# Arthur151/ROMP

Measured on NVIDIA H100. Metric: frames/sec 512x512 ROMP-HRNet32 (whole hot path), higher is better.
Workload: dtype bf16

## Files before the change

romp_b200/csrc/conv_tc.cu:

```cuda
#include <mutex>

#include "conv_tc.cuh"
#include "tc_device.cuh"

namespace b200romp {

thread_local int g_tc_pdl_override = -1;

constexpr int kTcThreads = 384;
constexpr int kMaxRings = 2;

__host__ __device__ constexpr int s2_row_bytes(int cin, int eb) { return cin * eb >= 512 ? 64 : (cin * eb < 128 ? cin * eb : 128); }

__host__ __device__ constexpr int tc_num_rings(int stages) { return stages >= 4 ? kMaxRings : 1; }
__host__ __device__ constexpr int tc_ring_size(int stages, int ring) { return tc_num_rings(stages) == 1 ? stages : (stages + 1 - ring) / 2; }
__host__ __device__ constexpr int tc_ring_base(int stages, int ring) { return ring ? (stages + 1) / 2 : 0; }

template <int MODE, int CIN, int NT, int EB>
struct TcCfg {
  static constexpr bool S2 = MODE == 2;
  static constexpr int KS = MODE == 1 ? 1 : 3;
  static constexpr int TAPS = KS * KS;
  static constexpr int PAD = KS / 2;
  static constexpr int ROWB = S2 ? s2_row_bytes(CIN, EB) : tc_row_bytes(KS, CIN, EB);
  static constexpr int CW = ROWB / EB;
  static constexpr int KCH = CIN / CW;
  static constexpr int KSTEPS = ROWB / 32;
  static constexpr uint32_t LAYOUT = tc_layout(ROWB);
  static constexpr int HW_ = 8 + 2 * PAD;
  static constexpr int HH = 16 + 2 * PAD;
  __host__ __device__ static constexpr int BH(int i) { return i < 2 ? 17 : 16; }
  __host__ __device__ static constexpr int BW(int i) { return (i & 1) ? 8 : 9; }
  __host__ __device__ static constexpr int SUB_BYTES(int i) { return (BH(i) * BW(i) * ROWB + 1023) / 1024 * 1024; }
  __host__ __device__ static constexpr int SUB_OFF(int i) { return i == 0 ? 0 : SUB_OFF(i - 1) + SUB_BYTES(i - 1); }
  static constexpr int STAGE_PAYLOAD = S2 ? (17 * 9 + 17 * 8 + 16 * 9 + 16 * 8) * ROWB : HH * HW_ * ROWB;
  static constexpr int STAGE_BYTES = S2 ? SUB_OFF(3) + SUB_BYTES(3) : (STAGE_PAYLOAD + 1023) / 1024 * 1024;
  static constexpr int BTILE = NT * ROWB;
  static constexpr int B_BYTES = TAPS * KCH * BTILE;
  static constexpr bool FOLDABLE = MODE == 3 && CIN == 64 && NT == 64 && EB == 2;
};

template <int MODE, int CIN, int NT, int EB, bool GENERIC>
__global__ void __launch_bounds__(kTcThreads, 1)
conv_tc_kernel(const __grid_constant__ CUtensorMap tmap, const __grid_constant__ S2Maps s2maps, const ConvParams p,
               const uint8_t* __restrict__ wpack, int tiles_x, int tiles_y, int num_tiles, int stages, unsigned kmask) {
  using Cfg = TcCfg<MODE, CIN, NT, EB>;
  extern __shared__ uint8_t smem_raw[];
  uint8_t* smem = reinterpret_cast<uint8_t*>((reinterpret_cast<uintptr_t>(smem_raw) + 1023) & ~(uintptr_t)1023);
  uint8_t* sB = smem;
  uint8_t* sA = smem + Cfg::B_BYTES;
  uint64_t* full = reinterpret_cast<uint64_t*>(sA + (size_t)stages * Cfg::STAGE_BYTES);
  uint64_t* empty = full + stages;
  uint64_t* b_full = empty + stages;

  const int warp = threadIdx.x >> 5;
  if (threadIdx.x == 0) {
    for (int i = 0; i < stages; ++i) {
      mbar_init(&full[i], 1);
      mbar_init(&empty[i], 4);
    }
    mbar_init(b_full, 1);
    fence_barrier_init();
  }
  __syncthreads();
  pdl_trigger();
  const int per_frame = tiles_x * tiles_y;
  const int nrings = tc_num_rings(stages);

  if (warp == 0) {
    if (elect_one()) {
      mbar_arrive_expect_tx(b_full, Cfg::B_BYTES);
      const uint8_t* wsrc = wpack + (size_t)blockIdx.y * Cfg::B_BYTES;
      for (int i = 0; i < Cfg::TAPS * Cfg::KCH; ++i)
        bulk_copy_g2s(sB + (size_t)i * Cfg::BTILE, wsrc + (size_t)i * Cfg::BTILE, Cfg::BTILE, b_full);
      pdl_wait();
      const uint64_t pol = l2_policy_stream();
      int stage = 0, stage_other = 0;
      uint32_t phase = 0, phase_other = 0;
      int it = 0;
      for (int tile = blockIdx.x; tile < num_tiles; tile += gridDim.x, ++it) {
        const int n = tile / per_frame, rem = tile % per_frame;
        const int y0 = (rem / tiles_x) * 16, x0 = (rem % tiles_x) * 8;
        const int ring = nrings == 2 ? (it & 1) : 0, rbase = tc_ring_base(stages, ring), rsize = tc_ring_size(stages, ring);
        for (int c = 0; c < Cfg::KCH; ++c) {
          const int sidx = rbase + stage;
          mbar_wait(&empty[sidx], phase ^ 1);
          mbar_arrive_expect_tx(&full[sidx], Cfg::STAGE_PAYLOAD);
          uint8_t* dst = sA + (size_t)sidx * Cfg::STAGE_BYTES;
          if constexpr (Cfg::S2) {
#pragma unroll
            for (int i = 0; i < 4; ++i) {
              const int ph = i < 2 ? 1 : 0, pw = (i & 1) ? 0 : 1;
              tma_load_5d(dst + Cfg::SUB_OFF(i), &s2maps.m[i], &full[sidx], pw * p.in_C + p.in_c_off + c * Cfg::CW, x0 - pw, ph,
                          y0 - ph, n, pol);
            }
          } else {
            tma_load_4d(dst, &tmap, &full[sidx], c * Cfg::CW, x0 - Cfg::PAD, y0 - Cfg::PAD, n, pol);
          }
          if (++stage == rsize) { stage = 0; phase ^= 1; }
        }
        if (nrings == 2) { const int ts = stage; stage = stage_other; stage_other = ts; const uint32_t tp = phase; phase = phase_other; phase_other = tp; }
      }
    }
  } else if (warp >= 4 && (warp >> 2) <= nrings) {
    const int g = (warp >> 2) - 1, t = threadIdx.x & 127, wlane = threadIdx.x & 31;
    pdl_wait();
    mbar_wait(b_full, 0);
    const uint32_t b_base = smem_u32(sB);
    const int rbase = tc_ring_base(stages, g), rsize = tc_ring_size(stages, g);
    int stage = 0;
    uint32_t phase = 0;
    for (int tile = blockIdx.x + g * gridDim.x; tile < num_tiles; tile += nrings * gridDim.x) {
      const int n = tile / per_frame, rem = tile % per_frame;
      const int y0 = (rem / tiles_x) * 16, x0 = (rem % tiles_x) * 8;
      float acc[2][NT / 2];
#pragma unroll
      for (int h = 0; h < 2; ++h)
#pragma unroll
        for (int j = 0; j < NT / 2; ++j) acc[h][j] = 0.f;
      uint32_t scale_d = 0;
      int prev = -1;
      for (int c = 0; c < Cfg::KCH; ++c) {
        const int sidx = rbase + stage;
        mbar_wait(&full[sidx], phase);
        uint8_t* a_stage = sA + (size_t)sidx * Cfg::STAGE_BYTES;
        if constexpr (EB == 4) {
          tf32_round_smem(a_stage, Cfg::STAGE_BYTES, t, 128);
          fence_proxy_async();
          wg_bar_sync(1 + g);
        }
        const uint32_t a_base = smem_u32(a_stage);
        wgmma_fence();
#pragma unroll
        for (int tap = 0; tap < Cfg::TAPS; ++tap) {
          const int r = tap / Cfg::KS, s = tap % Cfg::KS;
          uint32_t a_tap, sbo;
          if constexpr (Cfg::S2) {
            const int sub = (r != 1 ? 0 : 2) + (s != 1 ? 0 : 1);
            const int bw = Cfg::BW(sub);
            a_tap = a_base + (uint32_t)(Cfg::SUB_OFF(sub) + ((r == 2 ? bw : 0) + (s == 2 ? 1 : 0)) * Cfg::ROWB);
            sbo = bw * Cfg::ROWB;
          } else {
            a_tap = a_base + (uint32_t)((r * Cfg::HW_ + s) * Cfg::ROWB);
            sbo = Cfg::HW_ * Cfg::ROWB;
          }
          const uint32_t b_tap = b_base + (uint32_t)((tap * Cfg::KCH + c) * Cfg::BTILE);
#pragma unroll
          for (int k = 0; k < Cfg::KSTEPS; ++k) {
            if (Cfg::FOLDABLE && !((kmask >> (tap * 2 + (k * 2) / Cfg::KSTEPS)) & 1u)) continue;
            const uint64_t bdesc = make_smem_desc(b_tap + k * 32, 8 * Cfg::ROWB, Cfg::LAYOUT);
            wgmma_any<NT, EB>(acc[0], make_smem_desc(a_tap + k * 32, sbo, Cfg::LAYOUT), bdesc, scale_d);
            wgmma_any<NT, EB>(acc[1], make_smem_desc(a_tap + 8 * sbo + k * 32, sbo, Cfg::LAYOUT), bdesc, scale_d);
            scale_d = 1;
          }
        }
        wgmma_commit();
        if (prev >= 0) {
          wgmma_wait<1>();
          if (wlane == 0) mbar_arrive(&empty[prev]);
        }
        prev = sidx;
        if (++stage == rsize) { stage = 0; phase ^= 1; }
      }
      wgmma_wait<0>();
      if (wlane == 0) mbar_arrive(&empty[prev]);
      wg_epilogue<NT, GENERIC ? kEpiGeneric : kEpiNhwc>(p, acc, p.bias, n, y0, x0, blockIdx.y * NT, t);
    }
  }
}

PFN_encodeTiled tc_get_encode() {
  static PFN_encodeTiled fn = nullptr;
  static std::once_flag once;
  std::call_once(once, [] {
    void* ptr = nullptr;
    cudaDriverEntryPointQueryResult qres;
    if (cudaGetDriverEntryPoint("cuTensorMapEncodeTiled", &ptr, cudaEnableDefault, &qres) == cudaSuccess &&
        qres == cudaDriverEntryPointSuccess)
      fn = reinterpret_cast<PFN_encodeTiled>(ptr);
  });
  return fn;
}

int tc_encode_tiled(CUtensorMap* map, CUtensorMapDataType dtype, int rank, const void* base, const cuuint64_t* dims,
                    const cuuint64_t* strides, const cuuint32_t* box, CUtensorMapSwizzle swizzle, const char* tag) {
  PFN_encodeTiled encode = tc_get_encode();
  if (!encode) {
    set_error("%s: cuTensorMapEncodeTiled is unavailable", tag);
    return B200ROMP_ECUDA;
  }
  const cuuint32_t estr[5] = {1, 1, 1, 1, 1};
  const CUresult cr = encode(map, dtype, rank, const_cast<void*>(base), dims, strides, box, estr, CU_TENSOR_MAP_INTERLEAVE_NONE,
                             swizzle, CU_TENSOR_MAP_L2_PROMOTION_L2_128B, CU_TENSOR_MAP_FLOAT_OOB_FILL_NONE);
  if (cr != CUDA_SUCCESS) {
    set_error("%s: cuTensorMapEncodeTiled failed with %d", tag, (int)cr);
    return B200ROMP_ECUDA;
  }
  return B200ROMP_OK;
}

int tc_encode_nhwc_input(CUtensorMap* map, const ConvParams& p, int eb, int box_c, int box_w, int box_h, CUtensorMapSwizzle swizzle,
                         const char* tag) {
  const cuuint64_t dims[4] = {(cuuint64_t)p.cin, (cuuint64_t)p.Win, (cuuint64_t)p.Hin, (cuuint64_t)p.B};
  const cuuint64_t strides[3] = {(cuuint64_t)p.in_C * eb, (cuuint64_t)p.Win * p.in_C * eb, (cuuint64_t)p.Hin * p.Win * p.in_C * eb};
  const cuuint32_t box[4] = {(cuuint32_t)box_c, (cuuint32_t)box_w, (cuuint32_t)box_h, 1};
  return tc_encode_tiled(map, eb == 2 ? CU_TENSOR_MAP_DATA_TYPE_BFLOAT16 : CU_TENSOR_MAP_DATA_TYPE_FLOAT32, 4,
                         static_cast<const uint8_t*>(p.in) + (size_t)p.in_c_off * eb, dims, strides, box, swizzle, tag);
}

float tc_round_tf32_host(float w) {
  uint32_t u;
  memcpy(&u, &w, 4);
  if ((u & 0x7F800000u) != 0x7F800000u) u = (u + 0x1000u) & ~0x1FFFu;
  float r;
  memcpy(&r, &u, 4);
  return r;
}

std::vector<uint8_t> tc_pack_image(const float* w_oihw, int cin, int cout, int taps, int nt, int rowb, int eb) {
  const int cw = rowb / eb, kch = cin / cw, ntiles = (cout + nt - 1) / nt, per16 = 16 / eb;
  std::vector<uint8_t> img((size_t)ntiles * taps * kch * nt * rowb, 0);
  for (int j = 0; j < ntiles; ++j)
    for (int t = 0; t < taps; ++t)
      for (int c = 0; c < kch; ++c) {
        uint8_t* tile = img.data() + (((size_t)j * taps + t) * kch + c) * nt * rowb;
        for (int n = 0; n < nt; ++n)
          for (int k = 0; k < cw; ++k) {
            const int co = j * nt + n, ci = c * cw + k;
            if (co >= cout) continue;
            const float w = w_oihw[((size_t)co * cin + ci) * taps + t];
            const int chunk16 = k / per16;
            const int phase = rowb == 128 ? (n & 7) : ((n >> 1) & 3);
            const size_t byte = (size_t)n * rowb + (size_t)((chunk16 ^ phase) * 16) + (k % per16) * eb;
            if (eb == 2) { const __nv_bfloat16 b = __float2bfloat16_rn(w); memcpy(tile + byte, &b, 2); }
            else { const float f = tc_round_tf32_host(w); memcpy(tile + byte, &f, 4); }
          }
      }
  return img;
}

int tc_pack_weights(const float* w_oihw, int cin, int cout, int taps, int nt, void** d_out, std::vector<void*>* allocs, int rowb, int eb) {
  const std::vector<uint8_t> img = tc_pack_image(w_oihw, cin, cout, taps, nt, rowb, eb);
  *d_out = upload(img.data(), img.size(), allocs);
  return *d_out ? B200ROMP_OK : B200ROMP_ECUDA;
}

std::string TcConvPlan::describe() const {
  char buf[128];
  snprintf(buf, sizeof(buf), " [tc%s k%d v%d nt%d grid %dx%d smem %d stages %d%s]", eb == 4 ? "-tf32" : "", kind / 10, kind % 10, nt, grid_x,
           grid_y, smem_bytes, stages, kmask != 0xFFFFFFFFu ? " pixel-pairs" : "");
  return buf;
}

static bool tc_s2_supported(const ConvParams& p) {
  if ((p.in_dtype != B200ROMP_BF16 && p.in_dtype != B200ROMP_F32) || p.input_norm || p.out_nchw || p.pow_channel >= 0) return false;
  const int eb = p.in_dtype == B200ROMP_F32 ? 4 : 2;
  if (eb == 4 && (p.out_dtype != B200ROMP_F32 || (p.res != nullptr && p.res_dtype != B200ROMP_F32))) return false;
  if (p.cin != 32 && p.cin != 64 && p.cin != 128 && p.cin != 256) return false;
  if (eb == 4 && p.cin == 256) return false;
  if (p.in_C % 8 != 0 || p.in_c_off % 8 != 0) return false;
  if (p.cout % 32 != 0 || p.Hin % 2 != 0 || p.Win % 2 != 0) return false;
  if (p.Hout % 16 != 0 || p.Wout % 8 != 0 || p.Hout * 2 != p.Hin || p.Wout * 2 != p.Win) return false;
  if (p.out_C % 8 != 0 || p.out_c_off % 8 != 0) return false;
  if (p.res != nullptr && (p.res_C % 8 != 0 || p.res_c_off % 8 != 0)) return false;
  if ((reinterpret_cast<uintptr_t>(p.in) & 15) != 0) return false;
  return true;
}

static bool tc_shape_supported(const ConvParams& p, int ksize, int stride) {
  if (stride == 2 && ksize == 3) return tc_s2_supported(p);
  if (stride != 1 || (ksize != 1 && ksize != 3)) return false;
  if ((p.in_dtype != B200ROMP_BF16 && p.in_dtype != B200ROMP_F32) || p.input_norm) return false;
  if (p.in_dtype == B200ROMP_F32 && (p.out_dtype != B200ROMP_F32 || (p.res != nullptr && p.res_dtype != B200ROMP_F32))) return false;
  if (p.cin != 32 && p.cin != 64 && p.cin != 128 && p.cin != 256) return false;
  if (p.Hout % 16 != 0 || p.Wout % 8 != 0) return false;
  if (p.in_C % 8 != 0 || p.in_c_off % 8 != 0) return false;
  if (p.out_nchw) {
    if (p.out_dtype != B200ROMP_F32 || p.up != 1 || p.res != nullptr) return false;
    return (reinterpret_cast<uintptr_t>(p.in) & 15) == 0;
  }
  if (p.pow_channel >= 0 || p.cout % 32 != 0) return false;
  if (p.out_C % 8 != 0 || p.out_c_off % 8 != 0) return false;
  if (p.res != nullptr && (p.res_C % 8 != 0 || p.res_c_off % 8 != 0)) return false;
  if ((reinterpret_cast<uintptr_t>(p.in) & 15) != 0) return false;
  return true;
}

static int tc_rowb(int ksize, int stride, int cin, int eb) { return stride == 2 ? s2_row_bytes(cin, eb) : tc_row_bytes(ksize, cin, eb); }

static bool tc_tile(const ConvParams& p, int ksize, int stride, TcConvPlan* plan) {
  const int eb = p.in_dtype == B200ROMP_F32 ? 4 : 2;
  const int rowb = tc_rowb(ksize, stride, p.cin, eb), kch = p.cin / (rowb / eb);
  const int budget = 227 * 1024 - 1024  - 1024 ;
  auto bbytes = [&](int n) { return ksize * ksize * kch * n * rowb; };
  int nt = (p.cout % 64 == 0) ? 64 : 32;
  int stage_bytes, stages;
  if (stride == 2) {
    auto sub_bytes = [&](int i) { return ((i < 2 ? 17 : 16) * ((i & 1) ? 8 : 9) * rowb + 1023) / 1024 * 1024; };
    stage_bytes = sub_bytes(0) + sub_bytes(1) + sub_bytes(2) + sub_bytes(3);
    if (nt == 64 && bbytes(64) + 2 * stage_bytes > budget && bbytes(32) + 2 * stage_bytes <= budget) nt = 32;
    if (nt == 64 && bbytes(64) + stage_bytes > budget) nt = 32;
    if (bbytes(nt) + stage_bytes > budget) return false;
    stages = std::min(4, (budget - bbytes(nt)) / stage_bytes);
  } else {
    const int hh = 16 + 2 * (ksize / 2), hw = 8 + 2 * (ksize / 2);
    stage_bytes = (hh * hw * rowb + 1023) / 1024 * 1024;
    if (bbytes(nt) + 3 * stage_bytes > budget && nt == 64) nt = 32;
    if (bbytes(nt) + 2 * stage_bytes > budget && nt == 32) nt = 16;
    if (bbytes(nt) + 2 * stage_bytes > budget) return false;
    stages = std::min((budget - bbytes(nt)) / stage_bytes, 8);
  }
  plan->kind = stride == 2 ? 32 : ksize * 10;
  plan->eb = eb;
  plan->cin = p.cin; plan->cout = p.cout; plan->nt = nt;
  plan->stages = stages;
  plan->smem_bytes = bbytes(nt) + stages * stage_bytes + 1024 + 1024;
  return true;
}

bool tc_conv_supported(const ConvParams& p, int ksize, int stride) {
  TcConvPlan plan;
  return tc_shape_supported(p, ksize, stride) && tc_tile(p, ksize, stride, &plan);
}

template <int MODE, int CIN, int NT, int EB>
static int launch_inst(const TcConvPlan& plan, const ConvParams& p, cudaStream_t stream, bool set_attr_only) {
  if (set_attr_only) {
    B2R_CUDA_OK(cudaFuncSetAttribute(conv_tc_kernel<MODE, CIN, NT, EB, true>, cudaFuncAttributeMaxDynamicSharedMemorySize, 227 * 1024));
    B2R_CUDA_OK(cudaFuncSetAttribute(conv_tc_kernel<MODE, CIN, NT, EB, false>, cudaFuncAttributeMaxDynamicSharedMemorySize, 227 * 1024));
    return B200ROMP_OK;
  }
  auto kern = p.cout % NT == 0 && tc_nhwc_out(p, p.cout) ? conv_tc_kernel<MODE, CIN, NT, EB, false> : conv_tc_kernel<MODE, CIN, NT, EB, true>;
  const int tiles_x = p.Wout / 8, tiles_y = p.Hout / 16;
  const int num_tiles = tiles_x * tiles_y * p.B;
  dim3 grid(std::min(plan.grid_x, num_tiles), plan.grid_y);
  B2R_CUDA_OK(tc_launch(kern, grid, kTcThreads, plan.smem_bytes, stream, plan.tmap_in, plan.tmap_s2, p,
                        reinterpret_cast<const uint8_t*>(plan.d_wpack), tiles_x, tiles_y, num_tiles, plan.stages, plan.kmask));
  return B200ROMP_OK;
}

static int dispatch(const TcConvPlan& plan, const ConvParams& p, cudaStream_t stream, bool attr) {
  const int mode = plan.kind == 32 ? 2 : plan.kind / 10;
#define B2R_CASE(M, C, N, E) \
  if (mode == M && plan.cin == C && plan.nt == N && plan.eb == E) return launch_inst<M, C, N, E>(plan, p, stream, attr);
  B2R_CASE(3, 32, 32, 2) B2R_CASE(3, 32, 64, 2) B2R_CASE(3, 64, 32, 2) B2R_CASE(3, 64, 64, 2) B2R_CASE(3, 128, 32, 2) B2R_CASE(3, 128, 64, 2)
  B2R_CASE(3, 256, 32, 2) B2R_CASE(3, 256, 64, 2)
  B2R_CASE(1, 32, 32, 2) B2R_CASE(1, 32, 64, 2) B2R_CASE(1, 64, 32, 2) B2R_CASE(1, 64, 64, 2) B2R_CASE(1, 128, 32, 2) B2R_CASE(1, 128, 64, 2)
  B2R_CASE(1, 256, 32, 2) B2R_CASE(1, 256, 64, 2)
  B2R_CASE(2, 32, 32, 2) B2R_CASE(2, 32, 64, 2) B2R_CASE(2, 64, 32, 2) B2R_CASE(2, 64, 64, 2) B2R_CASE(2, 128, 32, 2) B2R_CASE(2, 256, 32, 2)
  B2R_CASE(3, 32, 32, 4) B2R_CASE(3, 32, 64, 4) B2R_CASE(3, 64, 32, 4) B2R_CASE(3, 64, 64, 4) B2R_CASE(3, 128, 32, 4) B2R_CASE(3, 256, 16, 4)
  B2R_CASE(1, 32, 32, 4) B2R_CASE(1, 32, 64, 4) B2R_CASE(1, 64, 32, 4) B2R_CASE(1, 64, 64, 4) B2R_CASE(1, 128, 32, 4) B2R_CASE(1, 128, 64, 4)
  B2R_CASE(1, 256, 32, 4) B2R_CASE(1, 256, 64, 4)
  B2R_CASE(2, 32, 32, 4) B2R_CASE(2, 32, 64, 4) B2R_CASE(2, 64, 32, 4) B2R_CASE(2, 128, 32, 4)
#undef B2R_CASE
  set_error("conv_tc: no instantiation for mode %d cin%d nt%d eb%d", mode, plan.cin, plan.nt, plan.eb);
  return B200ROMP_EINVAL;
}

int tc_conv_prepare(const ConvParams& p, int ksize, int stride, const float* w_oihw, int sm_count, TcConvPlan* plan,
                    std::vector<void*>* allocs) {
  if (!tc_tile(p, ksize, stride, plan)) {
    set_error("conv_tc: k%d s%d cin%d does not fit shared memory", ksize, stride, p.cin);
    return B200ROMP_EINVAL;
  }
  const int eb = plan->eb, rowb = tc_rowb(ksize, stride, p.cin, eb), cw = rowb / eb;
  plan->grid_y = (p.cout + plan->nt - 1) / plan->nt;
  plan->grid_x = std::max(1, sm_count / plan->grid_y);
  int rc = tc_pack_weights(w_oihw, p.cin, p.cout, ksize * ksize, plan->nt, &plan->d_wpack, allocs, rowb, eb);
  if (rc) return rc;
  const CUtensorMapSwizzle swizzle = rowb == 128 ? CU_TENSOR_MAP_SWIZZLE_128B : CU_TENSOR_MAP_SWIZZLE_64B;
  if (stride == 2) {
    const cuuint64_t C = (cuuint64_t)p.in_C;
    const cuuint64_t gdim[5] = {2 * C, (cuuint64_t)p.Win / 2, 2, (cuuint64_t)p.Hin / 2, (cuuint64_t)p.B};
    const cuuint64_t E = (cuuint64_t)eb;
    const cuuint64_t gstr[4] = {2 * C * E, (cuuint64_t)p.Win * C * E, 2 * (cuuint64_t)p.Win * C * E, (cuuint64_t)p.Hin * p.Win * C * E};
    const CUtensorMapDataType dtype = eb == 2 ? CU_TENSOR_MAP_DATA_TYPE_BFLOAT16 : CU_TENSOR_MAP_DATA_TYPE_FLOAT32;
    for (int i = 0; i < 4; ++i) {
      const cuuint32_t box[5] = {(cuuint32_t)cw, (cuuint32_t)((i & 1) ? 8 : 9), 1, (cuuint32_t)(i < 2 ? 17 : 16), 1};
      rc = tc_encode_tiled(&plan->tmap_s2.m[i], dtype, 5, p.in, gdim, gstr, box, swizzle, "conv_tc (stride 2)");
      if (rc) return rc;
    }
  } else {
    const int hh = 16 + 2 * (ksize / 2), hw = 8 + 2 * (ksize / 2);
    rc = tc_encode_nhwc_input(&plan->tmap_in, p, eb, cw, hw, hh, swizzle, "conv_tc");
    if (rc) return rc;
  }
  return dispatch(*plan, p, nullptr, true);
}

int tc_conv_launch(const TcConvPlan& plan, const ConvParams& p, cudaStream_t stream) { return dispatch(plan, p, stream, false); }

}
```

romp_b200/csrc/tc_device.cuh:

```cuda
#pragma once
#include <cuda.h>

#include <vector>

#include "conv_tc.cuh"

namespace b200romp {

__device__ __forceinline__ uint32_t smem_u32(const void* p) { return (uint32_t)__cvta_generic_to_shared(p); }

__device__ __forceinline__ void mbar_init(uint64_t* bar, uint32_t count) {
  asm volatile("mbarrier.init.shared::cta.b64 [%0], %1;" ::"r"(smem_u32(bar)), "r"(count) : "memory");
}
__device__ __forceinline__ void mbar_arrive_expect_tx(uint64_t* bar, uint32_t bytes) {
  asm volatile("mbarrier.arrive.expect_tx.shared::cta.b64 _, [%0], %1;" ::"r"(smem_u32(bar)), "r"(bytes) : "memory");
}
__device__ __forceinline__ void mbar_arrive(uint64_t* bar) {
  asm volatile("mbarrier.arrive.shared::cta.b64 _, [%0];" ::"r"(smem_u32(bar)) : "memory");
}
__device__ __forceinline__ bool mbar_try_wait(uint64_t* bar, uint32_t parity) {
  uint32_t ok;
  asm volatile(
      "{\n\t.reg .pred p;\n\t"
      "mbarrier.try_wait.parity.shared::cta.b64 p, [%1], %2;\n\t"
      "selp.b32 %0, 1, 0, p;\n\t}"
      : "=r"(ok)
      : "r"(smem_u32(bar)), "r"(parity)
      : "memory");
  return ok != 0;
}
__device__ __forceinline__ void mbar_wait(uint64_t* bar, uint32_t parity) {
  if (mbar_try_wait(bar, parity)) return;
  const long long t0 = clock64();
  while (!mbar_try_wait(bar, parity)) {
    if (clock64() - t0 > 4000000000LL) __trap();
  }
}
__device__ __forceinline__ bool elect_one() {
  uint32_t pred;
  asm volatile("{\n\t.reg .pred p;\n\telect.sync _|p, 0xffffffff;\n\tselp.b32 %0, 1, 0, p;\n\t}" : "=r"(pred));
  return pred != 0;
}
__device__ __forceinline__ void pdl_trigger() { asm volatile("griddepcontrol.launch_dependents;" ::: "memory"); }
__device__ __forceinline__ void pdl_wait() { asm volatile("griddepcontrol.wait;" ::: "memory"); }
__device__ __forceinline__ void fence_barrier_init() { asm volatile("fence.mbarrier_init.release.cluster;" ::: "memory"); }
__device__ __forceinline__ void fence_proxy_async() { asm volatile("fence.proxy.async.shared::cta;" ::: "memory"); }
__device__ __forceinline__ void wg_bar_sync(int id) { asm volatile("bar.sync %0, 128;" ::"r"(id) : "memory"); }

__device__ __forceinline__ uint64_t l2_policy_stream() {
  uint64_t pol;
  asm volatile("createpolicy.fractional.L2::evict_normal.b64 %0, 1.0;" : "=l"(pol));
  return pol;
}
__device__ __forceinline__ void tma_load_3d(void* dst, const CUtensorMap* map, uint64_t* bar, int c0, int c1, int c2, uint64_t pol) {
  asm volatile(
      "cp.async.bulk.tensor.3d.shared::cluster.global.mbarrier::complete_tx::bytes.L2::cache_hint [%0], [%1, {%3, %4, %5}], [%2], %6;"
      ::"r"(smem_u32(dst)), "l"(map), "r"(smem_u32(bar)), "r"(c0), "r"(c1), "r"(c2), "l"(pol)
      : "memory");
}
__device__ __forceinline__ void tma_load_4d(void* dst, const CUtensorMap* map, uint64_t* bar, int c0, int c1, int c2, int c3, uint64_t pol) {
  asm volatile(
      "cp.async.bulk.tensor.4d.shared::cluster.global.mbarrier::complete_tx::bytes.L2::cache_hint [%0], [%1, {%3, %4, %5, %6}], [%2], %7;"
      ::"r"(smem_u32(dst)), "l"(map), "r"(smem_u32(bar)), "r"(c0), "r"(c1), "r"(c2), "r"(c3), "l"(pol)
      : "memory");
}
__device__ __forceinline__ void tma_load_5d(void* dst, const CUtensorMap* map, uint64_t* bar, int c0, int c1, int c2, int c3,
                                            int c4, uint64_t pol) {
  asm volatile(
      "cp.async.bulk.tensor.5d.shared::cluster.global.mbarrier::complete_tx::bytes.L2::cache_hint [%0], [%1, {%3, %4, %5, %6, %7}], [%2], %8;"
      ::"r"(smem_u32(dst)), "l"(map), "r"(smem_u32(bar)), "r"(c0), "r"(c1), "r"(c2), "r"(c3), "r"(c4), "l"(pol)
      : "memory");
}
__device__ __forceinline__ void bulk_copy_g2s(void* dst, const void* src, uint32_t bytes, uint64_t* bar) {
  asm volatile("cp.async.bulk.shared::cluster.global.mbarrier::complete_tx::bytes [%0], [%1], %2, [%3];"
               ::"r"(smem_u32(dst)), "l"(src), "r"(bytes), "r"(smem_u32(bar))
               : "memory");
}

__device__ __forceinline__ void wgmma_fence() { asm volatile("wgmma.fence.sync.aligned;" ::: "memory"); }
__device__ __forceinline__ void wgmma_commit() { asm volatile("wgmma.commit_group.sync.aligned;" ::: "memory"); }
template <int N>
__device__ __forceinline__ void wgmma_wait() { asm volatile("wgmma.wait_group.sync.aligned %0;" ::"n"(N) : "memory"); }

#define B2R_WG_R8(i) "+f"(d[i + 0]), "+f"(d[i + 1]), "+f"(d[i + 2]), "+f"(d[i + 3]), "+f"(d[i + 4]), "+f"(d[i + 5]), "+f"(d[i + 6]), "+f"(d[i + 7])
__device__ __forceinline__ void wgmma_n16(float (&d)[8], uint64_t a, uint64_t b, uint32_t scale_d, bool tf32) {
  if (!tf32)
    asm volatile(
        "{\n\t.reg .pred p;\n\tsetp.ne.b32 p, %10, 0;\n\t"
        "wgmma.mma_async.sync.aligned.m64n16k16.f32.bf16.bf16 {%0, %1, %2, %3, %4, %5, %6, %7}, %8, %9, p, 1, 1, 0, 0;\n\t}"
        : B2R_WG_R8(0)
        : "l"(a), "l"(b), "r"(scale_d)
        : "memory");
  else
    asm volatile(
        "{\n\t.reg .pred p;\n\tsetp.ne.b32 p, %10, 0;\n\t"
        "wgmma.mma_async.sync.aligned.m64n16k8.f32.tf32.tf32 {%0, %1, %2, %3, %4, %5, %6, %7}, %8, %9, p, 1, 1;\n\t}"
        : B2R_WG_R8(0)
        : "l"(a), "l"(b), "r"(scale_d)
        : "memory");
}
__device__ __forceinline__ void wgmma_n32(float (&d)[16], uint64_t a, uint64_t b, uint32_t scale_d, bool tf32) {
  if (!tf32)
    asm volatile(
        "{\n\t.reg .pred p;\n\tsetp.ne.b32 p, %18, 0;\n\t"
        "wgmma.mma_async.sync.aligned.m64n32k16.f32.bf16.bf16 {%0, %1, %2, %3, %4, %5, %6, %7, %8, %9, %10, %11, %12, %13, %14, %15}, "
        "%16, %17, p, 1, 1, 0, 0;\n\t}"
        : B2R_WG_R8(0), B2R_WG_R8(8)
        : "l"(a), "l"(b), "r"(scale_d)
        : "memory");
  else
    asm volatile(
        "{\n\t.reg .pred p;\n\tsetp.ne.b32 p, %18, 0;\n\t"
        "wgmma.mma_async.sync.aligned.m64n32k8.f32.tf32.tf32 {%0, %1, %2, %3, %4, %5, %6, %7, %8, %9, %10, %11, %12, %13, %14, %15}, "
        "%16, %17, p, 1, 1;\n\t}"
        : B2R_WG_R8(0), B2R_WG_R8(8)
        : "l"(a), "l"(b), "r"(scale_d)
        : "memory");
}
__device__ __forceinline__ void wgmma_n64(float (&d)[32], uint64_t a, uint64_t b, uint32_t scale_d, bool tf32) {
  if (!tf32)
    asm volatile(
        "{\n\t.reg .pred p;\n\tsetp.ne.b32 p, %34, 0;\n\t"
        "wgmma.mma_async.sync.aligned.m64n64k16.f32.bf16.bf16 {%0, %1, %2, %3, %4, %5, %6, %7, %8, %9, %10, %11, %12, %13, %14, "
        "%15, %16, %17, %18, %19, %20, %21, %22, %23, %24, %25, %26, %27, %28, %29, %30, %31}, %32, %33, p, 1, 1, 0, 0;\n\t}"
        : B2R_WG_R8(0), B2R_WG_R8(8), B2R_WG_R8(16), B2R_WG_R8(24)
        : "l"(a), "l"(b), "r"(scale_d)
        : "memory");
  else
    asm volatile(
        "{\n\t.reg .pred p;\n\tsetp.ne.b32 p, %34, 0;\n\t"
        "wgmma.mma_async.sync.aligned.m64n64k8.f32.tf32.tf32 {%0, %1, %2, %3, %4, %5, %6, %7, %8, %9, %10, %11, %12, %13, %14, "
        "%15, %16, %17, %18, %19, %20, %21, %22, %23, %24, %25, %26, %27, %28, %29, %30, %31}, %32, %33, p, 1, 1;\n\t}"
        : B2R_WG_R8(0), B2R_WG_R8(8), B2R_WG_R8(16), B2R_WG_R8(24)
        : "l"(a), "l"(b), "r"(scale_d)
        : "memory");
}
__device__ __forceinline__ void wgmma_n128_bf16(float (&d)[64], uint64_t a, uint64_t b, uint32_t scale_d) {
  asm volatile(
      "{\n\t.reg .pred p;\n\tsetp.ne.b32 p, %66, 0;\n\t"
      "wgmma.mma_async.sync.aligned.m64n128k16.f32.bf16.bf16 {%0, %1, %2, %3, %4, %5, %6, %7, %8, %9, %10, %11, %12, %13, %14, "
      "%15, %16, %17, %18, %19, %20, %21, %22, %23, %24, %25, %26, %27, %28, %29, %30, %31, %32, %33, %34, %35, %36, %37, %38, "
      "%39, %40, %41, %42, %43, %44, %45, %46, %47, %48, %49, %50, %51, %52, %53, %54, %55, %56, %57, %58, %59, %60, %61, %62, "
      "%63}, %64, %65, p, 1, 1, 0, 0;\n\t}"
      : B2R_WG_R8(0), B2R_WG_R8(8), B2R_WG_R8(16), B2R_WG_R8(24), B2R_WG_R8(32), B2R_WG_R8(40), B2R_WG_R8(48), B2R_WG_R8(56)
      : "l"(a), "l"(b), "r"(scale_d)
      : "memory");
}
__device__ __forceinline__ void wgmma_n192_bf16(float (&d)[96], uint64_t a, uint64_t b, uint32_t scale_d) {
  asm volatile(
      "{\n\t.reg .pred p;\n\tsetp.ne.b32 p, %98, 0;\n\t"
      "wgmma.mma_async.sync.aligned.m64n192k16.f32.bf16.bf16 {%0, %1, %2, %3, %4, %5, %6, %7, %8, %9, %10, %11, %12, %13, %14, "
      "%15, %16, %17, %18, %19, %20, %21, %22, %23, %24, %25, %26, %27, %28, %29, %30, %31, %32, %33, %34, %35, %36, %37, %38, "
      "%39, %40, %41, %42, %43, %44, %45, %46, %47, %48, %49, %50, %51, %52, %53, %54, %55, %56, %57, %58, %59, %60, %61, %62, "
      "%63, %64, %65, %66, %67, %68, %69, %70, %71, %72, %73, %74, %75, %76, %77, %78, %79, %80, %81, %82, %83, %84, %85, %86, "
      "%87, %88, %89, %90, %91, %92, %93, %94, %95}, %96, %97, p, 1, 1, 0, 0;\n\t}"
      : B2R_WG_R8(0), B2R_WG_R8(8), B2R_WG_R8(16), B2R_WG_R8(24), B2R_WG_R8(32), B2R_WG_R8(40), B2R_WG_R8(48), B2R_WG_R8(56),
        B2R_WG_R8(64), B2R_WG_R8(72), B2R_WG_R8(80), B2R_WG_R8(88)
      : "l"(a), "l"(b), "r"(scale_d)
      : "memory");
}
#undef B2R_WG_R8
template <int NT, int EB>
__device__ __forceinline__ void wgmma_any(float (&d)[NT / 2], uint64_t a, uint64_t b, uint32_t scale_d) {
  if constexpr (NT == 64) wgmma_n64(d, a, b, scale_d, EB == 4);
  else if constexpr (NT == 32) wgmma_n32(d, a, b, scale_d, EB == 4);
  else wgmma_n16(d, a, b, scale_d, EB == 4);
}

constexpr uint32_t kSw128 = 1, kSw64 = 2;
__device__ __forceinline__ uint64_t make_smem_desc(uint32_t addr, uint32_t sbo_bytes, uint32_t layout) {
  return (uint64_t)((addr & 0x3FFFF) >> 4) | ((uint64_t)1 << 16) | ((uint64_t)(sbo_bytes >> 4) << 32) | ((uint64_t)layout << 62);
}
__host__ __device__ constexpr uint32_t tc_layout(int row_bytes) { return row_bytes == 128 ? kSw128 : kSw64; }

__host__ __device__ constexpr int tc_row_bytes(int ksize, int cin, int eb) {
  return (ksize == 3 && cin >= 128) ? 64 : (cin * eb < 128 ? cin * eb : 128);
}

__device__ __forceinline__ uint32_t tf32_rna(uint32_t x) {
  uint32_t y;
  asm("cvt.rna.tf32.f32 %0, %1;" : "=r"(y) : "r"(x));
  return y;
}
__device__ __forceinline__ void tf32_round_smem(uint8_t* base, int bytes, int t, int nthreads) {
  const uint32_t s0 = smem_u32(base);
  for (int off = t * 16; off < bytes; off += nthreads * 16) {
    uint32_t a, b, c, d;
    asm volatile("ld.shared.v4.b32 {%0, %1, %2, %3}, [%4];" : "=r"(a), "=r"(b), "=r"(c), "=r"(d) : "r"(s0 + off));
    a = tf32_rna(a); b = tf32_rna(b); c = tf32_rna(c); d = tf32_rna(d);
    asm volatile("st.shared.v4.b32 [%4], {%0, %1, %2, %3};" ::"r"(a), "r"(b), "r"(c), "r"(d), "r"(s0 + off) : "memory");
  }
}

__device__ __forceinline__ void wg_store2(const ConvParams& p, int n, int oy, int ox, int co, float v0, float v1) {
  if (p.out_nchw || p.pow_channel >= 0 || co + 2 > p.cout) {
    const float v[2] = {v0, v1};
    conv_epilogue_store<2>(p, n, oy, ox, co, v);
    return;
  }
  const int up = p.up, Hf = p.Hout * up, Wf = p.Wout * up;
  for (int dy = 0; dy < up; ++dy) {
    for (int dx = 0; dx < up; ++dx) {
      const int fy = oy * up + dy, fx = ox * up + dx;
      const size_t pix = ((size_t)n * Hf + fy) * Wf + fx;
      float a = v0, b = v1;
      if (p.res != nullptr) {
        const size_t ri = ((size_t)(p.res_broadcast ? 0 : n) * Hf + fy) * Wf + fx;
        const size_t idx = ri * p.res_C + p.res_c_off + co;
        if (p.res_dtype == B200ROMP_BF16) {
          const __nv_bfloat162 r = *reinterpret_cast<const __nv_bfloat162*>(reinterpret_cast<const __nv_bfloat16*>(p.res) + idx);
          a += __low2float(r); b += __high2float(r);
        } else {
          const float2 r = *reinterpret_cast<const float2*>(reinterpret_cast<const float*>(p.res) + idx);
          a += r.x; b += r.y;
        }
      }
      if (p.relu) { a = fmaxf(a, 0.f); b = fmaxf(b, 0.f); }
      const size_t oi = pix * p.out_C + p.out_c_off + co;
      if (p.out_dtype == B200ROMP_BF16)
        *reinterpret_cast<__nv_bfloat162*>(reinterpret_cast<__nv_bfloat16*>(p.out) + oi) = __floats2bfloat162_rn(a, b);
      else
        *reinterpret_cast<float2*>(reinterpret_cast<float*>(p.out) + oi) = make_float2(a, b);
    }
  }
}

__host__ __device__ __forceinline__ bool tc_nhwc_out(const ConvParams& p, int co_end) {
  return p.up == 1 && !p.out_nchw && p.pow_channel < 0 && co_end <= p.cout;
}

__device__ __forceinline__ float2 res_pair(uint32_t r) {
  const __nv_bfloat162 v = *reinterpret_cast<const __nv_bfloat162*>(&r);
  return make_float2(__low2float(v), __high2float(v));
}
__device__ __forceinline__ float2 res_pair(float2 r) { return r; }

template <int NT, typename RT, int ROWS = (NT / 8) * (int)sizeof(RT) <= 16 ? 4 : (NT / 8) * (int)sizeof(RT) <= 32 ? 2 : 1>
__device__ __forceinline__ void wg_epilogue_nhwc(const ConvParams& p, const float (&acc)[2][NT / 2], int n, int y0, int x0, int co0,
                                                 int w, int l, bool linear) {
  const int dpix = linear ? 8 : p.Wout;
  auto pix0 = [&](int frame) -> size_t {
    return linear ? ((size_t)frame * p.Hout + y0) * p.Wout + x0 + 16 * w + (l >> 2)
                  : ((size_t)frame * p.Hout + y0 + 2 * w) * p.Wout + x0 + (l >> 2);
  };
  const int c = co0 + 2 * (l & 3);
  const uint8_t* rbase = nullptr;
  int rstep = 0;
  if (p.res != nullptr) {
    rbase = reinterpret_cast<const uint8_t*>(p.res) + (pix0(p.res_broadcast ? 0 : n) * p.res_C + p.res_c_off + c) * (sizeof(RT) / 2);
    rstep = dpix * p.res_C * (int)(sizeof(RT) / 2);
  }
  const int ob = p.out_dtype == B200ROMP_BF16 ? 2 : 4;
  uint8_t* obase = reinterpret_cast<uint8_t*>(p.out) + (pix0(n) * p.out_C + p.out_c_off + c) * ob;
  const int ostep = dpix * p.out_C * ob;
#pragma unroll
  for (int q0 = 0; q0 < 4; q0 += ROWS) {
    RT rv[ROWS][NT / 8];
    if (p.res != nullptr) {
#pragma unroll
      for (int qq = 0; qq < ROWS; ++qq) {
        const int q = q0 + qq;
        const RT* r = reinterpret_cast<const RT*>(rbase + (8 * (q >> 1) + (q & 1)) * rstep);
#pragma unroll
        for (int j = 0; j < NT / 8; ++j) rv[qq][j] = r[4 * j];
      }
    }
#pragma unroll
    for (int qq = 0; qq < ROWS; ++qq) {
      const int q = q0 + qq, h = q >> 1, e = q & 1;
      uint8_t* o = obase + (8 * h + e) * ostep;
#pragma unroll
      for (int j = 0; j < NT / 8; ++j) {
        float a = acc[h][4 * j + 2 * e], b = acc[h][4 * j + 2 * e + 1];
        if (p.res != nullptr) { const float2 r = res_pair(rv[qq][j]); a += r.x; b += r.y; }
        if (p.relu) { a = fmaxf(a, 0.f); b = fmaxf(b, 0.f); }
        if (ob == 2) reinterpret_cast<__nv_bfloat162*>(o)[4 * j] = __floats2bfloat162_rn(a, b);
        else reinterpret_cast<float2*>(o)[4 * j] = make_float2(a, b);
      }
    }
  }
}

constexpr int kEpiNhwc = 0, kEpiGeneric = 1, kEpiAny = 2;
template <int NT, int PATH = kEpiAny>
__device__ __forceinline__ void wg_epilogue(const ConvParams& p, float (&acc)[2][NT / 2], const float* __restrict__ bias, int n,
                                            int y0, int x0, int co0, int wg_thread, bool linear = false) {
  const int w = wg_thread >> 5, l = wg_thread & 31;
  if (PATH == kEpiNhwc || (PATH == kEpiAny && tc_nhwc_out(p, co0 + NT))) {
#pragma unroll
    for (int j = 0; j < NT / 8; ++j) {
      const int c = co0 + 8 * j + 2 * (l & 3);
      const float b0 = __ldg(bias + c), b1 = __ldg(bias + c + 1);
#pragma unroll
      for (int h = 0; h < 2; ++h) {
        acc[h][4 * j] += b0; acc[h][4 * j + 1] += b1; acc[h][4 * j + 2] += b0; acc[h][4 * j + 3] += b1;
      }
    }
    if (p.res != nullptr && p.res_dtype == B200ROMP_F32) wg_epilogue_nhwc<NT, float2>(p, acc, n, y0, x0, co0, w, l, linear);
    else wg_epilogue_nhwc<NT, uint32_t>(p, acc, n, y0, x0, co0, w, l, linear);
    return;
  }
  if constexpr (PATH != kEpiNhwc) {
#pragma unroll
    for (int h = 0; h < 2; ++h) {
#pragma unroll
      for (int j = 0; j < NT / 8; ++j) {
        const int c = co0 + 8 * j + 2 * (l & 3);
        const float b0 = __ldg(bias + c), b1 = __ldg(bias + c + 1);
#pragma unroll
        for (int e = 0; e < 2; ++e) {
          const int m = 64 * h + 16 * w + (l >> 2) + 8 * e;
          wg_store2(p, n, linear ? y0 : y0 + (m >> 3), linear ? x0 + m : x0 + (m & 7), c, acc[h][4 * j + 2 * e] + b0,
                    acc[h][4 * j + 2 * e + 1] + b1);
        }
      }
    }
  }
}

template <typename... KArgs, typename... Args>
static inline cudaError_t tc_launch(void (*kern)(KArgs...), dim3 grid, int threads, int smem_bytes, cudaStream_t stream, Args&&... args) {
  static const bool pdl_default = [] { const char* e = getenv("B200ROMP_NO_PDL"); return !(e && e[0] == '1'); }();
  const bool pdl = pdl_default && g_tc_pdl_override != 0;
  cudaLaunchConfig_t cfg = {};
  cfg.gridDim = grid;
  cfg.blockDim = dim3(threads);
  cfg.dynamicSmemBytes = (size_t)smem_bytes;
  cfg.stream = stream;
  cudaLaunchAttribute at[1];
  at[0].id = cudaLaunchAttributeProgrammaticStreamSerialization;
  at[0].val.programmaticStreamSerializationAllowed = 1;
  cfg.attrs = at;
  cfg.numAttrs = pdl ? 1 : 0;
  return cudaLaunchKernelEx(&cfg, kern, static_cast<KArgs>(args)...);
}

typedef CUresult (*PFN_encodeTiled)(CUtensorMap*, CUtensorMapDataType, cuuint32_t, void*, const cuuint64_t*, const cuuint64_t*,
                                    const cuuint32_t*, const cuuint32_t*, CUtensorMapInterleave, CUtensorMapSwizzle,
                                    CUtensorMapL2promotion, CUtensorMapFloatOOBfill);
PFN_encodeTiled tc_get_encode();
int tc_encode_tiled(CUtensorMap* map, CUtensorMapDataType dtype, int rank, const void* base, const cuuint64_t* dims,
                    const cuuint64_t* strides, const cuuint32_t* box, CUtensorMapSwizzle swizzle, const char* tag);
int tc_encode_nhwc_input(CUtensorMap* map, const ConvParams& p, int eb, int box_c, int box_w, int box_h, CUtensorMapSwizzle swizzle,
                         const char* tag);
std::vector<uint8_t> tc_pack_image(const float* w_oihw, int cin, int cout, int taps, int nt, int rowb, int eb);
int tc_pack_weights(const float* w_oihw, int cin, int cout, int taps, int nt, void** d_out, std::vector<void*>* allocs, int rowb, int eb);
float tc_round_tf32_host(float w);

}
```

Baseline: 3589.

## Add swapped weights-as-A wgmma path and streamed-weight kernel for 256-channel 3x3 convs

Result: faster. 3720 (median of 6 runs) (+3.7%).

```diff
diff --git a/romp_b200/csrc/conv_tc.cu b/romp_b200/csrc/conv_tc.cu
--- a/romp_b200/csrc/conv_tc.cu
+++ b/romp_b200/csrc/conv_tc.cu
@@ -40,11 +40,12 @@
   static constexpr bool FOLDABLE = MODE == 3 && CIN == 64 && NT == 64 && EB == 2;
 };
 
-template <int MODE, int CIN, int NT, int EB, bool GENERIC>
+template <int MODE, int CIN, int NT, int EB, bool GENERIC, bool SWAP = false>
 __global__ void __launch_bounds__(kTcThreads, 1)
 conv_tc_kernel(const __grid_constant__ CUtensorMap tmap, const __grid_constant__ S2Maps s2maps, const ConvParams p,
                const uint8_t* __restrict__ wpack, int tiles_x, int tiles_y, int num_tiles, int stages, unsigned kmask) {
   using Cfg = TcCfg<MODE, CIN, NT, EB>;
+  static_assert(!SWAP || (MODE == 3 && NT == 64 && EB == 2 && !GENERIC), "the swapped plan is bf16 3x3 stride 1, NHWC, M = 64");
   extern __shared__ uint8_t smem_raw[];
   uint8_t* smem = reinterpret_cast<uint8_t*>((reinterpret_cast<uintptr_t>(smem_raw) + 1023) & ~(uintptr_t)1023);
   uint8_t* sB = smem;
@@ -149,8 +150,12 @@
           for (int k = 0; k < Cfg::KSTEPS; ++k) {
             if (Cfg::FOLDABLE && !((kmask >> (tap * 2 + (k * 2) / Cfg::KSTEPS)) & 1u)) continue;
             const uint64_t bdesc = make_smem_desc(b_tap + k * 32, 8 * Cfg::ROWB, Cfg::LAYOUT);
-            wgmma_any<NT, EB>(acc[0], make_smem_desc(a_tap + k * 32, sbo, Cfg::LAYOUT), bdesc, scale_d);
-            wgmma_any<NT, EB>(acc[1], make_smem_desc(a_tap + 8 * sbo + k * 32, sbo, Cfg::LAYOUT), bdesc, scale_d);
+            if constexpr (SWAP) {
+              wgmma_n128_bf16(*reinterpret_cast<float(*)[64]>(&acc[0][0]), bdesc, make_smem_desc(a_tap + k * 32, sbo, Cfg::LAYOUT), scale_d);
+            } else {
+              wgmma_any<NT, EB>(acc[0], make_smem_desc(a_tap + k * 32, sbo, Cfg::LAYOUT), bdesc, scale_d);
+              wgmma_any<NT, EB>(acc[1], make_smem_desc(a_tap + 8 * sbo + k * 32, sbo, Cfg::LAYOUT), bdesc, scale_d);
+            }
             scale_d = 1;
           }
         }
@@ -164,7 +169,105 @@
       }
       wgmma_wait<0>();
       if (wlane == 0) mbar_arrive(&empty[prev]);
-      wg_epilogue<NT, GENERIC ? kEpiGeneric : kEpiNhwc>(p, acc, p.bias, n, y0, x0, blockIdx.y * NT, t);
+      if constexpr (SWAP) {
+        if (p.res != nullptr && p.res_dtype == B200ROMP_F32)
+          wg_epilogue_swap<float2>(p, *reinterpret_cast<float(*)[64]>(&acc[0][0]), n, y0, x0, blockIdx.y * NT, t);
+        else
+          wg_epilogue_swap<uint32_t>(p, *reinterpret_cast<float(*)[64]>(&acc[0][0]), n, y0, x0, blockIdx.y * NT, t);
+      } else {
+        wg_epilogue<NT, GENERIC ? kEpiGeneric : kEpiNhwc>(p, acc, p.bias, n, y0, x0, blockIdx.y * NT, t);
+      }
+    }
+  }
+}
+
+constexpr int kStrmCin = 256, kStrmKch = kStrmCin / 32, kStrmRowB = 64, kStrmHalo = 18;
+constexpr int kStrmWBytes = 9 * 64 * kStrmRowB;
+constexpr int kStrmHaloPayload = kStrmHalo * kStrmHalo * kStrmRowB;
+constexpr int kStrmStageBytes = kStrmWBytes + (kStrmHaloPayload + 1023) / 1024 * 1024;
+constexpr int kStrmStages = 3;
+constexpr int kStrmSmem = kStrmStages * kStrmStageBytes + 1024  + 1024 ;
+static_assert(kStrmSmem <= 227 * 1024, "streamed-weight stages do not fit shared memory");
+
+__global__ void __launch_bounds__(kTcThreads, 1)
+conv_tc_stream_kernel(const __grid_constant__ CUtensorMap tmap, const ConvParams p, const uint8_t* __restrict__ wpack, int tiles_x,
+                      int tiles_y, int nslabs, int num_items) {
+  extern __shared__ uint8_t smem_raw[];
+  uint8_t* smem = reinterpret_cast<uint8_t*>((reinterpret_cast<uintptr_t>(smem_raw) + 1023) & ~(uintptr_t)1023);
+  uint64_t* full = reinterpret_cast<uint64_t*>(smem + kStrmStages * kStrmStageBytes);
+  uint64_t* empty = full + kStrmStages;
+  const int warp = threadIdx.x >> 5;
+  if (threadIdx.x == 0) {
+    for (int i = 0; i < kStrmStages; ++i) {
+      mbar_init(&full[i], 1);
+      mbar_init(&empty[i], 8);
+    }
+    fence_barrier_init();
+  }
+  __syncthreads();
+  pdl_trigger();
+  const int per_frame = tiles_x * tiles_y;
+
+  if (warp == 0) {
+    if (elect_one()) {
+      pdl_wait();
+      const uint64_t pol = l2_policy_stream();
+      int stage = 0;
+      uint32_t phase = 0;
+      for (int item = blockIdx.x; item < num_items; item += gridDim.x) {
+        const int tile = item / nslabs, slab = item % nslabs;
+        const int n = tile / per_frame, rem = tile % per_frame;
+        const int y0 = (rem / tiles_x) * 16, x0 = (rem % tiles_x) * 16;
+        for (int c = 0; c < kStrmKch; ++c) {
+          mbar_wait(&empty[stage], phase ^ 1);
+          mbar_arrive_expect_tx(&full[stage], kStrmWBytes + kStrmHaloPayload);
+          uint8_t* dst = smem + (size_t)stage * kStrmStageBytes;
+          bulk_copy_g2s(dst, wpack + ((size_t)slab * kStrmKch + c) * kStrmWBytes, kStrmWBytes, &full[stage]);
+          tma_load_4d(dst + kStrmWBytes, &tmap, &full[stage], c * 32, x0 - 1, y0 - 1, n, pol);
+          if (++stage == kStrmStages) { stage = 0; phase ^= 1; }
+        }
+      }
+    }
+  } else if (warp >= 4) {
+    const int g = (warp >> 2) - 1, t = threadIdx.x & 127, wlane = threadIdx.x & 31;
+    pdl_wait();
+    int stage = 0;
+    uint32_t phase = 0;
+    for (int item = blockIdx.x; item < num_items; item += gridDim.x) {
+      const int tile = item / nslabs, slab = item % nslabs;
+      const int n = tile / per_frame, rem = tile % per_frame;
+      const int y0 = (rem / tiles_x) * 16, x0 = (rem % tiles_x) * 16;
+      float acc[64];
+#pragma unroll
+      for (int j = 0; j < 64; ++j) acc[j] = 0.f;
+      uint32_t scale_d = 0;
+      int prev = -1;
+      for (int c = 0; c < kStrmKch; ++c) {
+        mbar_wait(&full[stage], phase);
+        const uint32_t w_base = smem_u32(smem + (size_t)stage * kStrmStageBytes), a_base = w_base + kStrmWBytes;
+        wgmma_fence();
+#pragma unroll
+        for (int tap = 0; tap < 9; ++tap) {
+          const uint32_t a_tap = a_base + (uint32_t)(((tap / 3) * kStrmHalo + tap % 3 + 8 * g) * kStrmRowB);
+#pragma unroll
+          for (int k = 0; k < 2; ++k) {
+            wgmma_n128_bf16(acc, make_smem_desc(w_base + tap * 64 * kStrmRowB + k * 32, 8 * kStrmRowB, kSw64),
+                            make_smem_desc(a_tap + k * 32, kStrmHalo * kStrmRowB, kSw64), scale_d);
+            scale_d = 1;
+          }
+        }
+        wgmma_commit();
+        if (prev >= 0) {
+          wgmma_wait<1>();
+          if (wlane == 0) mbar_arrive(&empty[prev]);
+        }
+        prev = stage;
+        if (++stage == kStrmStages) { stage = 0; phase ^= 1; }
+      }
+      wgmma_wait<0>();
+      if (wlane == 0) mbar_arrive(&empty[prev]);
+      if (p.res != nullptr && p.res_dtype == B200ROMP_F32) wg_epilogue_swap<float2>(p, acc, n, y0, x0 + 8 * g, slab * 64, t);
+      else wg_epilogue_swap<uint32_t>(p, acc, n, y0, x0 + 8 * g, slab * 64, t);
     }
   }
 }
@@ -247,8 +350,8 @@
 
 std::string TcConvPlan::describe() const {
   char buf[128];
-  snprintf(buf, sizeof(buf), " [tc%s k%d v%d nt%d grid %dx%d smem %d stages %d%s]", eb == 4 ? "-tf32" : "", kind / 10, kind % 10, nt, grid_x,
-           grid_y, smem_bytes, stages, kmask != 0xFFFFFFFFu ? " pixel-pairs" : "");
+  snprintf(buf, sizeof(buf), " [tc%s k%d v%d nt%d grid %dx%d smem %d stages %d%s]%s", eb == 4 ? "-tf32" : "", kind / 10, kind % 10, nt,
+           grid_x, grid_y, smem_bytes, stages, kmask != 0xFFFFFFFFu ? " pixel-pairs" : "", kind == 31 ? " [tc-swap weights-as-A n128]" : kind == 34 ? " [tc-stream weights-as-A n128 tile 16x16]" : "");
   return buf;
 }
 
@@ -288,11 +391,24 @@
 
 static int tc_rowb(int ksize, int stride, int cin, int eb) { return stride == 2 ? s2_row_bytes(cin, eb) : tc_row_bytes(ksize, cin, eb); }
 
+static bool tc_stream_eligible(const ConvParams& p, int ksize, int stride) {
+  return ksize == 3 && stride == 1 && p.in_dtype == B200ROMP_BF16 && p.cin == kStrmCin && p.cout % 64 == 0 &&
+         p.out_dtype == B200ROMP_BF16 && tc_nhwc_out(p, p.cout) && p.Hout % 16 == 0 && p.Wout % 16 == 0;
+}
+
 static bool tc_tile(const ConvParams& p, int ksize, int stride, TcConvPlan* plan) {
   const int eb = p.in_dtype == B200ROMP_F32 ? 4 : 2;
   const int rowb = tc_rowb(ksize, stride, p.cin, eb), kch = p.cin / (rowb / eb);
   const int budget = 227 * 1024 - 1024  - 1024 ;
   auto bbytes = [&](int n) { return ksize * ksize * kch * n * rowb; };
+  if (tc_stream_eligible(p, ksize, stride)) {
+    plan->kind = 34;
+    plan->eb = 2;
+    plan->cin = p.cin; plan->cout = p.cout; plan->nt = 64;
+    plan->stages = kStrmStages;
+    plan->smem_bytes = kStrmSmem;
+    return true;
+  }
   int nt = (p.cout % 64 == 0) ? 64 : 32;
   int stage_bytes, stages;
   if (stride == 2) {
@@ -311,6 +427,9 @@
     stages = std::min((budget - bbytes(nt)) / stage_bytes, 8);
   }
   plan->kind = stride == 2 ? 32 : ksize * 10;
+  if (ksize == 3 && stride == 1 && eb == 2 && p.cin == 128 && p.cout == 128 && nt == 64 && p.out_dtype == B200ROMP_BF16 &&
+      tc_nhwc_out(p, p.cout))
+    plan->kind = 31;
   plan->eb = eb;
   plan->cin = p.cin; plan->cout = p.cout; plan->nt = nt;
   plan->stages = stages;
@@ -323,14 +442,19 @@
   return tc_shape_supported(p, ksize, stride) && tc_tile(p, ksize, stride, &plan);
 }
 
-template <int MODE, int CIN, int NT, int EB>
+template <int MODE, int CIN, int NT, int EB, bool SWAP = false>
 static int launch_inst(const TcConvPlan& plan, const ConvParams& p, cudaStream_t stream, bool set_attr_only) {
   if (set_attr_only) {
-    B2R_CUDA_OK(cudaFuncSetAttribute(conv_tc_kernel<MODE, CIN, NT, EB, true>, cudaFuncAttributeMaxDynamicSharedMemorySize, 227 * 1024));
-    B2R_CUDA_OK(cudaFuncSetAttribute(conv_tc_kernel<MODE, CIN, NT, EB, false>, cudaFuncAttributeMaxDynamicSharedMemorySize, 227 * 1024));
+    if constexpr (SWAP) {
+      B2R_CUDA_OK(cudaFuncSetAttribute(conv_tc_kernel<MODE, CIN, NT, EB, false, true>, cudaFuncAttributeMaxDynamicSharedMemorySize, 227 * 1024));
+    } else {
+      B2R_CUDA_OK(cudaFuncSetAttribute(conv_tc_kernel<MODE, CIN, NT, EB, true>, cudaFuncAttributeMaxDynamicSharedMemorySize, 227 * 1024));
+      B2R_CUDA_OK(cudaFuncSetAttribute(conv_tc_kernel<MODE, CIN, NT, EB, false>, cudaFuncAttributeMaxDynamicSharedMemorySize, 227 * 1024));
+    }
     return B200ROMP_OK;
   }
-  auto kern = p.cout % NT == 0 && tc_nhwc_out(p, p.cout) ? conv_tc_kernel<MODE, CIN, NT, EB, false> : conv_tc_kernel<MODE, CIN, NT, EB, true>;
+  auto kern = SWAP ? conv_tc_kernel<MODE, CIN, NT, EB, false, SWAP>
+                   : p.cout % NT == 0 && tc_nhwc_out(p, p.cout) ? conv_tc_kernel<MODE, CIN, NT, EB, false> : conv_tc_kernel<MODE, CIN, NT, EB, true>;
   const int tiles_x = p.Wout / 8, tiles_y = p.Hout / 16;
   const int num_tiles = tiles_x * tiles_y * p.B;
   dim3 grid(std::min(plan.grid_x, num_tiles), plan.grid_y);
@@ -341,6 +465,18 @@
 
 static int dispatch(const TcConvPlan& plan, const ConvParams& p, cudaStream_t stream, bool attr) {
   const int mode = plan.kind == 32 ? 2 : plan.kind / 10;
+  if (plan.kind == 34) {
+    if (attr) {
+      B2R_CUDA_OK(cudaFuncSetAttribute(conv_tc_stream_kernel, cudaFuncAttributeMaxDynamicSharedMemorySize, kStrmSmem));
+      return B200ROMP_OK;
+    }
+    const int tiles_x = p.Wout / 16, tiles_y = p.Hout / 16, nslabs = p.cout / 64;
+    const int num_items = tiles_x * tiles_y * p.B * nslabs;
+    B2R_CUDA_OK(tc_launch(conv_tc_stream_kernel, dim3(std::min(plan.grid_x, num_items)), kTcThreads, plan.smem_bytes, stream, plan.tmap_in,
+                          p, reinterpret_cast<const uint8_t*>(plan.d_wpack), tiles_x, tiles_y, nslabs, num_items));
+    return B200ROMP_OK;
+  }
+  if (plan.kind == 31 && plan.cin == 128 && plan.nt == 64 && plan.eb == 2) return launch_inst<3, 128, 64, 2, true>(plan, p, stream, attr);
 #define B2R_CASE(M, C, N, E) \
   if (mode == M && plan.cin == C && plan.nt == N && plan.eb == E) return launch_inst<M, C, N, E>(plan, p, stream, attr);
   B2R_CASE(3, 32, 32, 2) B2R_CASE(3, 32, 64, 2) B2R_CASE(3, 64, 32, 2) B2R_CASE(3, 64, 64, 2) B2R_CASE(3, 128, 32, 2) B2R_CASE(3, 128, 64, 2)
@@ -362,6 +498,22 @@
   if (!tc_tile(p, ksize, stride, plan)) {
     set_error("conv_tc: k%d s%d cin%d does not fit shared memory", ksize, stride, p.cin);
     return B200ROMP_EINVAL;
+  }
+  if (plan->kind == 34) {
+    const std::vector<uint8_t> img = tc_pack_image(w_oihw, p.cin, p.cout, 9, 64, kStrmRowB, 2);
+    std::vector<uint8_t> strm(img.size());
+    const size_t tile = 64 * kStrmRowB;
+    for (int j = 0; j < p.cout / 64; ++j)
+      for (int tap = 0; tap < 9; ++tap)
+        for (int c = 0; c < kStrmKch; ++c)
+          memcpy(strm.data() + (((size_t)j * kStrmKch + c) * 9 + tap) * tile, img.data() + (((size_t)j * 9 + tap) * kStrmKch + c) * tile, tile);
+    plan->d_wpack = upload(strm.data(), strm.size(), allocs);
+    if (!plan->d_wpack) return B200ROMP_ECUDA;
+    plan->grid_x = sm_count;
+    plan->grid_y = 1;
+    const int rc = tc_encode_nhwc_input(&plan->tmap_in, p, 2, 32, kStrmHalo, kStrmHalo, CU_TENSOR_MAP_SWIZZLE_64B, "conv_tc (streamed)");
+    if (rc) return rc;
+    return dispatch(*plan, p, nullptr, true);
   }
   const int eb = plan->eb, rowb = tc_rowb(ksize, stride, p.cin, eb), cw = rowb / eb;
   plan->grid_y = (p.cout + plan->nt - 1) / plan->nt;
diff --git a/romp_b200/csrc/tc_device.cuh b/romp_b200/csrc/tc_device.cuh
--- a/romp_b200/csrc/tc_device.cuh
+++ b/romp_b200/csrc/tc_device.cuh
@@ -318,6 +318,48 @@
   }
 }
 
+template <typename RT, int JB = sizeof(RT) == 4 ? 16 : 8>
+__device__ __forceinline__ void wg_epilogue_swap(const ConvParams& p, const float (&acc)[64], int n, int y0, int x0, int co0,
+                                                 int wg_thread) {
+  const int w = wg_thread >> 5, l = wg_thread & 31, odd = (l >> 2) & 1;
+  const int c = co0 + 16 * w + (l >> 2);
+  const float bias[2] = {__ldg(p.bias + c), __ldg(p.bias + c + 8)};
+  const int ch = c & ~1;
+  const size_t pix = ((size_t)n * p.Hout + y0) * p.Wout + x0 + 2 * (l & 3) + odd;
+  __nv_bfloat16* out = reinterpret_cast<__nv_bfloat16*>(p.out) + pix * p.out_C + p.out_c_off + ch;
+  const size_t ostep = (size_t)p.Wout * p.out_C;
+  const uint8_t* rbase = nullptr;
+  size_t rstep = 0;
+  if (p.res != nullptr) {
+    const size_t rpix = p.res_broadcast ? pix - (size_t)n * p.Hout * p.Wout : pix;
+    rbase = reinterpret_cast<const uint8_t*>(p.res) + (rpix * p.res_C + p.res_c_off + ch) * (sizeof(RT) / 2);
+    rstep = (size_t)p.Wout * p.res_C * (sizeof(RT) / 2);
+  }
+#pragma unroll
+  for (int j0 = 0; j0 < 16; j0 += JB) {
+    RT rv[JB][2];
+    if (p.res != nullptr) {
+#pragma unroll
+      for (int jj = 0; jj < JB; ++jj)
+#pragma unroll
+        for (int e = 0; e < 2; ++e) rv[jj][e] = reinterpret_cast<const RT*>(rbase + (j0 + jj) * rstep)[4 * e];
+    }
+#pragma unroll
+    for (int jj = 0; jj < JB; ++jj) {
+      const int j = j0 + jj;
+#pragma unroll
+      for (int e = 0; e < 2; ++e) {
+        const float v0 = acc[4 * j + 2 * e] + bias[e], v1 = acc[4 * j + 2 * e + 1] + bias[e];
+        const float recv = __shfl_xor_sync(0xffffffffu, odd ? v0 : v1, 4);
+        float a = odd ? recv : v0, b = odd ? v1 : recv;
+        if (p.res != nullptr) { const float2 r = res_pair(rv[jj][e]); a += r.x; b += r.y; }
+        if (p.relu) { a = fmaxf(a, 0.f); b = fmaxf(b, 0.f); }
+        *reinterpret_cast<__nv_bfloat162*>(out + j * ostep + 8 * e) = __floats2bfloat162_rn(a, b);
+      }
+    }
+  }
+}
+
 template <typename... KArgs, typename... Args>
 static inline cudaError_t tc_launch(void (*kern)(KArgs...), dim3 grid, int threads, int smem_bytes, cudaStream_t stream, Args&&... args) {
   static const bool pdl_default = [] { const char* e = getenv("B200ROMP_NO_PDL"); return !(e && e[0] == '1'); }();
```
